# ut-amrl/IV_SLAM

Measured on AMD Instinct MI355X. Metric: stereo pairs/s (extract+match+introspect) @1242×375, 1000 feat; 1/2/4/8 GPU, higher is better.
Workload: dtype u8 (ORB) + f32 via split-f16 MFMA (FCN); 1 GPU; configs[2]: 1242x375 stereo stream with introspection FCN cost-map forward (MFMA convs) gating keypoints, ORB extract + L/R Hamming match; width=1242, height=375, pairs_per_launch_sequence=128, distinct_pairs_per_gpu=512, nfeatures=1000, nlevels=8, parallelism=1 GPU

## Files before the change

### iv_slam_amd/csrc/ivf_fcn.hip

```cpp
#include <hip/hip_runtime.h>
#include <cmath>
#include <cstdarg>
#include <cstdio>
#include <cstdlib>
#include <cstring>
#include <string>
#include <vector>
#include "ivf_device.h"

#define ffail ivf::set_error

#include <type_traits>
namespace ivffcn {

#define FHIP(expr)                                                                                   \
    do { hipError_t e_ = (expr);                                                                      \
         if (e_ != hipSuccess) return ffail(IVF_E_NO_DEVICE, "%s failed: %s", #expr, hipGetErrorString(e_)); } while (0)

typedef float f32x16 __attribute__((ext_vector_type(16)));
typedef float v2f __attribute__((ext_vector_type(2)));
typedef _Float16 f16x8 __attribute__((ext_vector_type(8)));
typedef _Float16 f16x2 __attribute__((ext_vector_type(2)));
union HFrag { f16x8 v; uint4 q; uint32_t u[4]; };
typedef int i32x8 __attribute__((ext_vector_type(8)));
// ... 409 lines not shown
            if (tid + NT * k < NTAB4) ((float4*)sTP)[tid + NT * k] = t4[k];
#pragma unroll
        for (int k = 0; k < IT; k++)
            if (tid + NT * k < N4) *(float4*)&sX[dst[k]] = ok[k] ? v4[k] : make_float4(0.f, 0.f, 0.f, 0.f);
    }
    f32x16 accO;
#pragma unroll
    for (int q = 0; q < 16; q++) accO[q] = 0.f;
    __syncthreads();
    IRB_TIM(0);
    constexpr int TPW = (NTE + 7) / 8;
    HFrag xh[TPW][K16], xl[TPW][K16];
#pragma unroll
    for (int ti = 0; ti < TPW; ti++) {
        const int nc = min(32 * (wv + 8 * ti) + col, NPOS - 1);
        const float* base = sX + (nc / RW) * RP + nc % RW + 3;
#pragma unroll
        for (int st = 0; st < K16; st++)
#pragma unroll
            for (int jj = 0; jj < 4; jj++) {
                const int k0 = 16 * st + 8 * hh + 2 * jj;
                const float x0 = k0 < CIN ? base[k0 * XPL] : 0.f, x1 = k0 + 1 < CIN ? base[(k0 + 1) * XPL] : 0.f;
                split_pair(x0, x1, xh[ti][st].u[jj], xl[ti][st].u[jj]);
            }
    }
    IRB_TIM(1);
#pragma unroll 1
    for (int g = 0; g < NG; g++) {
        HFrag ph[2], pl[2];
        {
            float sc[16], sh[16];
#pragma unroll
            for (int r = 0; r < 16; r++) {
                const float* t = sT + (32 * g + (r & 3) + 8 * (r >> 2) + 4 * hh) * TP;
                sc[r] = t[0]; sh[r] = t[1];
            }
#pragma unroll
            for (int ti = 0; ti < TPW; ti++) {
                const int t = wv + 8 * ti;
                if (t >= NTE) break;
                const int n = 32 * t + col, nc = min(n, NPOS - 1);
                const int r_ = nc / RW, q_ = nc % RW;
                f32x16 acc;
#pragma unroll
                for (int q = 0; q < 16; q++) acc[q] = 0.f;
#pragma unroll
                for (int st = 0; st < K16; st++) {
                    acc = __builtin_amdgcn_mfma_f32_32x32x16_f16(el[st].v, xh[ti][st].v, acc, 0, 0, 0);
                    acc = __builtin_amdgcn_mfma_f32_32x32x16_f16(eh[st].v, xl[ti][st].v, acc, 0, 0, 0);
                    acc = __builtin_amdgcn_mfma_f32_32x32x16_f16(eh[st].v, xh[ti][st].v, acc, 0, 0, 0);
                }
                if (n < NPOS) {
                    const bool edgeWg = ry0 < 0 || rx0 < 0 || ry0 + RH > WI || rx0 + RW > WI;
                    if (!edgeWg) {
#pragma unroll
                        for (int r = 0; r < 16; r++)
                            sH[((r & 3) + 8 * (r >> 2) + 4 * hh) * HPL + n] = __builtin_amdgcn_fmed3f(__builtin_fmaf(acc[r], sc[r], sh[r]), 0.f, 6.f);
                    } else {
                        const bool inside = (unsigned)(ry0 + r_) < (unsigned)WI && (unsigned)(rx0 + q_) < (unsigned)WI;
#pragma unroll
                        for (int r = 0; r < 16; r++) {
                            const float v = __builtin_amdgcn_fmed3f(__builtin_fmaf(acc[r], sc[r], sh[r]), 0.f, 6.f);
                            sH[((r & 3) + 8 * (r >> 2) + 4 * hh) * HPL + n] = inside ? v : 0.f;
                        }
                    }
                }
            }
#ifdef IVF_IRB_ABL_FRAG
            if (g == 0)
#endif
            if (wv < NTP) {
#pragma unroll
                for (int st = 0; st < 2; st++) { ph[st].q = WqP[((2 * g + st) * 2 + 0) * 64 + lane]; pl[st].q = WqP[((2 * g + st) * 2 + 1) * 64 + lane]; }
            }
#ifndef IVF_IRB_ABL_FRAG
            {
                const int gn = g + 1 < NG ? g + 1 : 0;
#pragma unroll
                for (int st = 0; st < K16; st++) { eh[st].q = WqE[((st * NG + gn) * 2 + 0) * 64 + lane]; el[st].q = WqE[((st * NG + gn) * 2 + 1) * 64 + lane]; }
            }
#endif
        }
        IRB_TIM(2);
        __syncthreads();
        IRB_TIM(3);
        {
            const int chl = tid >> 4, sub = tid & 15;
            constexpr int PX = TW * TH / 16;
            const int oy = sub / (TW / PX), x0 = (sub % (TW / PX)) * PX;
            const float* tb = sT + (32 * g + chl) * TP;
            float wk[9];
#pragma unroll
            for (int k = 0; k < 9; k++) wk[k] = tb[2 + k];
            const float dsc = tb[11], dsh = tb[12];
            const float* hp = sH + chl * HPL + (oy * S) * RW + x0 * S;
            float o[PX];
#pragma unroll
            for (int p = 0; p < PX; p++) o[p] = 0.f;
#pragma unroll
            for (int ky = 0; ky < 3; ky++) {
                float row[(PX - 1) * S + 3];
#pragma unroll
                for (int k = 0; k < (PX - 1) * S + 3; k++) row[k] = hp[ky * RW + k];
#pragma unroll
                for (int kx = 0; kx < 3; kx++)
#pragma unroll
                    for (int p = 0; p < PX; p++) o[p] = __builtin_fmaf(wk[ky * 3 + kx], row[p * S + kx], o[p]);
            }
            float* dp = sD + chl * DPL + oy * TW + x0;
#pragma unroll
            for (int p = 0; p < PX; p++) dp[p] = __builtin_amdgcn_fmed3f(__builtin_fmaf(o[p], dsc, dsh), 0.f, 6.f);
        }
        IRB_TIM(4);
        __syncthreads();
        IRB_TIM(5);
        if (wv < NTP) {
            const float* src = sD + 32 * wv + col;
#pragma unroll
            for (int st = 0; st < 2; st++) {
                HFrag bh, bl;
#pragma unroll
                for (int jj = 0; jj < 4; jj++) {
                    const int k0 = 16 * st + 8 * hh + 2 * jj;
                    split_pair(src[k0 * DPL], src[(k0 + 1) * DPL], bh.u[jj], bl.u[jj]);
                }
                accO = __builtin_amdgcn_mfma_f32_32x32x16_f16(pl[st].v, bh.v, accO, 0, 0, 0);
                accO = __builtin_amdgcn_mfma_f32_32x32x16_f16(ph[st].v, bl.v, accO, 0, 0, 0);
                accO = __builtin_amdgcn_mfma_f32_32x32x16_f16(ph[st].v, bh.v, accO, 0, 0, 0);
            }
        }
        IRB_TIM(6);
    }
    if (wv < NTP) {
        const int n = 32 * wv + col, y = oy0 + n / TW, x = ox0 + n % TW;
        float amax = 0.f;
#pragma unroll
        for (int r = 0; r < 16; r++) {
            const int ch = (r & 3) + 8 * (r >> 2) + 4 * hh;
            if (ch >= COUT) continue;
            float v = __builtin_fmaf(accO[r], sPB[ch], sPB[32 + ch]);
            if (RES) v += sX[ch * XPL + (n / TW + 1) * RP + (n % TW + 1) + 3];
            range_note(amax, v);
            Y[(size_t)b * COUT * WO * WO + (ilOut ? ((size_t)y * COUT + ch) * WO : ((size_t)ch * WO + y) * WO) + x] = v;
        }
        range_flag(amax);
    }
#ifdef IVF_IRB_TIMING
    if (WI == IVF_IRB_TIMING && S == IVF_IRB_TIMING_S) {
        asm volatile("s_waitcnt vmcnt(0)" ::: "memory");
        IRB_TIM(7);
        if (tid == 0) { for (int i = 0; i < 8; i++) atomicAdd(&g_irbTim[i], tacc[i]); atomicAdd(&g_irbTim[8], 1ull); }
    }
#endif
}

template <int DIL, int CIN, int HID, int COUT, bool RES>
__global__ __launch_bounds__(512, 4) void k_fcn_irb64(const float* __restrict__ X, const uint4* __restrict__ WqE,
                                                  const float* __restrict__ se, const float* __restrict__ be,
                                                  const float* __restrict__ Wd, const float* __restrict__ sd,
                                                  const float* __restrict__ bd, const uint4* __restrict__ WqP,
                                                  const float* __restrict__ sp, const float* __restrict__ bp, float* __restrict__ Y)
{
    constexpr int NT = 512, WI = 64, TW = 32, TH = 2;
    constexpr int RW = TW + 2 * DIL, RH = TH + 2 * DIL, NPOS = RW * RH;
    constexpr int HPL = (NPOS + 3) / 4 * 4 + 4, DPL = TW * TH + 4;
    constexpr int K16 = (CIN + 15) / 16, NG = (HID + 31) / 32, NTE = (NPOS + 31) / 32, MT = (COUT + 31) / 32, TP = 13;
    static_assert(NTE <= 8, "one window tile per wave");
    static_assert(MT <= 4, "one output-channel tile per wave");
    __shared__ __attribute__((aligned(16))) float sH[32 * HPL];
    __shared__ __attribute__((aligned(16))) float sD[32 * DPL];
    __shared__ float sT[2][32 * TP];
    const int tid = threadIdx.x, b = blockIdx.z;
    const int ox0 = blockIdx.x * TW, oy0 = blockIdx.y * TH;
    const int rx0 = ox0 - DIL, ry0 = oy0 - DIL;
    const float* Xb = X + (size_t)b * CIN * WI * WI;
    const int wv = __builtin_amdgcn_readfirstlane(tid >> 6), lane = tid & 63, hh = lane >> 5, col = lane & 31;
    const float* tsrc; int tstride;
    {
        const int f = tid % TP;
        tsrc = f == 0 ? se : f == 1 ? be : f < 11 ? Wd + (f - 2) : f == 11 ? sd : bd;
        tstride = (f >= 2 && f < 11) ? 9 : 1;
    }
    auto fetch_table = [&](int g) {
        const int c = 32 * g + tid / TP;
        return (tid < 32 * TP && c < HID) ? tsrc[(size_t)c * tstride] : 0.f;
    };
    HFrag eh[K16], el[K16];
#pragma unroll
    for (int st = 0; st < K16; st++) { eh[st].q = WqE[((st * NG + 0) * 2 + 0) * 64 + lane]; el[st].q = WqE[((st * NG + 0) * 2 + 1) * 64 + lane]; }
    if (tid < 32 * TP) sT[0][tid] = fetch_table(0);
    const int n = 32 * wv + col, nc = min(n, NPOS - 1);
    const int r_ = nc / RW, q_ = nc % RW;
    const bool inside = (unsigned)(ry0 + r_) < (unsigned)WI && (unsigned)(rx0 + q_) < (unsigned)WI;
    HFrag xh[K16], xl[K16];
    {
        const float* src = Xb + (size_t)(inside ? ry0 + r_ : 0) * WI + (inside ? rx0 + q_ : 0);
        float xv[K16][8];
#pragma unroll
        for (int st = 0; st < K16; st++)
#pragma unroll
            for (int j = 0; j < 8; j++) {
                const int k = 16 * st + 8 * hh + j;
                xv[st][j] = k < CIN ? src[(size_t)k * WI * WI] : 0.f;
            }
#pragma unroll
        for (int st = 0; st < K16; st++)
#pragma unroll
            for (int jj = 0; jj < 4; jj++)
                split_pair(inside ? xv[st][2 * jj] : 0.f, inside ? xv[st][2 * jj + 1] : 0.f, xh[st].u[jj], xl[st].u[jj]);
    }
    f32x16 accO;
#pragma unroll
    for (int q = 0; q < 16; q++) accO[q] = 0.f;
    const int ntP = wv & 1, mtP = wv >> 1;
    __syncthreads();
#pragma unroll 1
    for (int g = 0; g < NG; g++) {
        const float* T = sT[g & 1];
        const float tnext = g + 1 < NG ? fetch_table(g + 1) : 0.f;
        if (wv < NTE) {
            f32x16 acc, acc1;
#pragma unroll
            for (int q = 0; q < 16; q++) { acc[q] = 0.f; acc1[q] = 0.f; }
#pragma unroll
            for (int st = 0; st < K16; st++) {
                acc1 = __builtin_amdgcn_mfma_f32_32x32x16_f16(el[st].v, xh[st].v, acc1, 0, 0, 0);
                acc = __builtin_amdgcn_mfma_f32_32x32x16_f16(eh[st].v, xh[st].v, acc, 0, 0, 0);
                acc1 = __builtin_amdgcn_mfma_f32_32x32x16_f16(eh[st].v, xl[st].v, acc1, 0, 0, 0);
            }
#pragma unroll
            for (int q = 0; q < 16; q++) acc[q] += acc1[q];
            if (n < NPOS) {
#pragma unroll
                for (int r = 0; r < 16; r++) {
                    const int cl = (r & 3) + 8 * (r >> 2) + 4 * hh;
                    const float v = __builtin_amdgcn_fmed3f(__builtin_fmaf(acc[r], T[cl * TP], T[cl * TP + 1]), 0.f, 6.f);
                    sH[cl * HPL + n] = inside ? v : 0.f;
                }
            }
        }
        if (g + 1 < NG) {
#pragma unroll
            for (int st = 0; st < K16; st++) { eh[st].q = WqE[((st * NG + g + 1) * 2 + 0) * 64 + lane]; el[st].q = WqE[((st * NG + g + 1) * 2 + 1) * 64 + lane]; }
        }
        __syncthreads();
        {
            const int chl = tid >> 4, sub = tid & 15;
            const int oy = sub >> 3, x0 = (sub & 7) * 4;
            const float* tb = T + chl * TP;
            float wk[9];
#pragma unroll
            for (int k = 0; k < 9; k++) wk[k] = tb[2 + k];
            const float dsc = tb[11], dsh = tb[12];
            const float* hp = sH + chl * HPL + oy * RW + x0;
            float o[4] = {0.f, 0.f, 0.f, 0.f};
#pragma unroll
            for (int ky = 0; ky < 3; ky++) {
                float row[4 + 2 * DIL];
#pragma unroll
                for (int k = 0; k < 4 + 2 * DIL; k++) row[k] = hp[ky * DIL * RW + k];
#pragma unroll
                for (int kx = 0; kx < 3; kx++)
#pragma unroll
                    for (int p = 0; p < 4; p++) o[p] = __builtin_fmaf(wk[ky * 3 + kx], row[p + kx * DIL], o[p]);
            }
            float* dp = sD + chl * DPL + oy * TW + x0;
#pragma unroll
            for (int p = 0; p < 4; p++) dp[p] = __builtin_amdgcn_fmed3f(__builtin_fmaf(o[p], dsc, dsh), 0.f, 6.f);
        }
        if (g + 1 < NG && tid < 32 * TP) sT[(g + 1) & 1][tid] = tnext;
        __syncthreads();
        if (mtP < MT) {
            HFrag ph[2], pl[2];
#pragma unroll
            for (int st = 0; st < 2; st++) {
                ph[st].q = WqP[(((2 * g + st) * MT + mtP) * 2 + 0) * 64 + lane];
                pl[st].q = WqP[(((2 * g + st) * MT + mtP) * 2 + 1) * 64 + lane];
            }
            const float* src = sD + 32 * ntP + col;
#pragma unroll
            for (int st = 0; st < 2; st++) {
                HFrag bh, bl;
#pragma unroll
                for (int jj = 0; jj < 4; jj++) {
                    const int k0 = 16 * st + 8 * hh + 2 * jj;
                    split_pair(src[k0 * DPL], src[(k0 + 1) * DPL], bh.u[jj], bl.u[jj]);
                }
                accO = __builtin_amdgcn_mfma_f32_32x32x16_f16(pl[st].v, bh.v, accO, 0, 0, 0);
                accO = __builtin_amdgcn_mfma_f32_32x32x16_f16(ph[st].v, bl.v, accO, 0, 0, 0);
                accO = __builtin_amdgcn_mfma_f32_32x32x16_f16(ph[st].v, bh.v, accO, 0, 0, 0);
            }
        }
    }
    if (mtP < MT) {
        const int m = 32 * ntP + col, y = oy0 + m / TW, x = ox0 + m % TW;
        float amax = 0.f;
#pragma unroll
        for (int r = 0; r < 16; r++) {
            const int ch = 32 * mtP + (r & 3) + 8 * (r >> 2) + 4 * hh;
            if (ch >= COUT) continue;
            float v = __builtin_fmaf(accO[r], sp[ch], bp[ch]);
            if (RES) v += Xb[((size_t)ch * WI + y) * WI + x];
            range_note(amax, v);
            Y[(((size_t)b * COUT + ch) * WI + y) * WI + x] = v;
        }
        range_flag(amax);
// ... 3392 lines not shown
}

int make_fused4(ivf_fcn* f, ivf_fcn::Fused4& F, const float* we, const std::vector<float>& scE, const std::vector<float>& shE, const float* wd,
                const std::vector<float>& scD, const std::vector<float>& shD, const float* wp, int cout, int cin = kF4Cin, int hid = kF4Hid)
{
    const int groups = hid / 16, ksteps = cin / 32;
    auto put = [](uint16_t* q, size_t frag, int lane, int j, float v) {
        const uint16_t hi = f32_to_f16(v), lo = f32_to_f16(v - f16_to_f32(hi));
        q[((frag + 0) * 64 + lane) * 8 + j] = hi; q[((frag + 1) * 64 + lane) * 8 + j] = lo;
    };
    F.cout = cout; F.tilesP = cout / 32;
    std::vector<float> qe((size_t)groups * ksteps * 2 * 64 * 4, 0.f), qp((size_t)groups * F.tilesP * 2 * 64 * 4, 0.f), par((size_t)hid * 12, 0.f);
    uint16_t* e16 = reinterpret_cast<uint16_t*>(qe.data()); uint16_t* p16 = reinterpret_cast<uint16_t*>(qp.data());
    for (int g = 0; g < groups; g++) {
        for (int s5 = 0; s5 < ksteps; s5++)
            for (int lane = 0; lane < 64; lane++)
                for (int j = 0; j < 8; j++)
                    put(e16, ((size_t)g * ksteps + s5) * 2, lane, j, we[(size_t)(16 * g + (lane & 15)) * cin + 32 * s5 + 8 * (lane >> 4) + j]);
        for (int t = 0; t < F.tilesP; t++)
            for (int lane = 0; lane < 64; lane++)
                for (int j = 0; j < 8; j++)
                    put(p16, ((size_t)g * F.tilesP + t) * 2, lane, j, wp[(size_t)(32 * t + (lane & 31)) * hid + 16 * g + 8 * (lane >> 5) + j]);
    }
    for (int c = 0; c < hid; c++) {
        for (int q = 0; q < 9; q++) par[(size_t)c * 12 + q] = wd[(size_t)c * 9 + q] * scD[c];
        par[(size_t)c * 12 + 9] = shD[c]; par[(size_t)c * 12 + 10] = scE[c]; par[(size_t)c * 12 + 11] = shE[c];
    }
    float *de = nullptr, *dp = nullptr;
    int rc;
    if ((rc = upload(f, qe, &de)) || (rc = upload(f, qp, &dp)) || (rc = upload(f, par, &F.dPar))) return rc;
    F.dWE = reinterpret_cast<uint4*>(de); F.dWP = reinterpret_cast<uint4*>(dp);
    if (IVF_F4_FP6_BUILT && cin == kF4Cin && hid == kF4Hid) {
        std::vector<float> q6((size_t)groups * 10 * 64 * 4, 0.f);
        uint32_t* d32 = reinterpret_cast<uint32_t*>(q6.data());
        uint16_t* d16 = reinterpret_cast<uint16_t*>(q6.data());
        for (int g = 0; g < groups; g++) {
            const size_t base = (size_t)g * 10 * 64 * 4;
            for (int s5 = 0; s5 < 5; s5++)
                for (int lane = 0; lane < 64; lane++)
                    for (int j = 0; j < 8; j++)
                        d16[(base + ((size_t)s5 * 64 + lane) * 4) * 2 + j] = f32_to_f16(we[(size_t)(16 * g + (lane & 15)) * cin + 32 * s5 + 8 * (lane >> 4) + j]);
            for (int c = 0; c < 3; c++)
                for (int lane = 0; lane < 64; lane++) {
                    int codes[32];
                    for (int e = 0; e < 32; e++) {
                        const int seg = e >> 3, j = e & 7, s5 = 2 * c + (seg >> 1);
                        float v = 0.f;
                        if (s5 < 5) {
                            const float w = we[(size_t)(16 * g + (lane & 15)) * cin + 32 * s5 + 8 * (lane >> 4) + j];
                            const float hi = f16_to_f32(f32_to_f16(w)), lo = f16_to_f32(f32_to_f16(w - hi));
                            v = (seg & 1) ? std::ldexp(hi, kF6SH) : std::ldexp(lo, kF6SH + 10);
                        }
                        codes[e] = enc6(v, true);
                    }
                    uint32_t six[6]; pack6(six, codes);
                    for (int q = 0; q < 4; q++) d32[base + ((size_t)(5 + c) * 64 + lane) * 4 + q] = six[q];
                    d32[base + (size_t)8 * 64 * 4 + ((size_t)c * 64 + lane) * 2 + 0] = six[4];
                    d32[base + (size_t)8 * 64 * 4 + ((size_t)c * 64 + lane) * 2 + 1] = six[5];
                }
        }
        float* d6 = nullptr;
        if ((rc = upload(f, q6, &d6))) return rc;
        F.dWE6 = reinterpret_cast<uint4*>(d6);
    }
    return IVF_OK;
}

int reserve_lds()
{
    struct { const void* fn; size_t lds; const char* name; } ks[] = {
        {reinterpret_cast<const void*>(&k_fcn_irbd2<32, 32, true, 1>), D2Cfg<32, 32, 1>::LDS, "k_fcn_irbd2<32,32,true,1>"},
        {reinterpret_cast<const void*>(&k_fcn_irbd2<32, 64, false, 1>), D2Cfg<32, 64, 1>::LDS, "k_fcn_irbd2<32,64,false,1>"},
        {reinterpret_cast<const void*>(&k_fcn_irbd2<64, 64, true>), D2Cfg<64, 64>::LDS, "k_fcn_irbd2<64,64,true>"},
        {reinterpret_cast<const void*>(&k_fcn_irbd2<64, 96, false>), D2Cfg<64, 96>::LDS, "k_fcn_irbd2<64,96,false>"},
        {reinterpret_cast<const void*>(&k_fcn_irbd2<96, 96, true>), D2Cfg<96, 96>::LDS, "k_fcn_irbd2<96,96,true>"},
        {reinterpret_cast<const void*>(&k_fcn_irbd2<96, 160, false>), D2Cfg<96, 160>::LDS, "k_fcn_irbd2<96,160,false>"},
        {reinterpret_cast<const void*>(&k_fcn_irbd4<true>), kF4Lds, "k_fcn_irbd4<true>"},
        {reinterpret_cast<const void*>(&k_fcn_irbd4<false>), kF4Lds, "k_fcn_irbd4<false>"},
#if IVF_F4_FP6_BUILT
        {reinterpret_cast<const void*>(&k_fcn_irbd4<true, false, true>), kF4Lds, "k_fcn_irbd4<true,fp6>"},
        {reinterpret_cast<const void*>(&k_fcn_irbd4<false, false, true>), kF4Lds, "k_fcn_irbd4<false,fp6>"},
        {reinterpret_cast<const void*>(&k_fcn_irbd4<false, true, true>), kF4Lds, "k_fcn_irbd4<split,fp6>"},
#endif
        {reinterpret_cast<const void*>(&k_fcn_irbd2<64, 64, true, 2, true>), D2Cfg<64, 64>::LDS, "k_fcn_irbd2<64,64,split>"},
        {reinterpret_cast<const void*>(&k_fcn_irbd2<64, 96, false, 2, true>), D2Cfg<64, 96>::LDS, "k_fcn_irbd2<64,96,split>"},
        {reinterpret_cast<const void*>(&k_fcn_irbd2<96, 96, true, 2, true>), D2Cfg<96, 96>::LDS, "k_fcn_irbd2<96,96,split>"},
        {reinterpret_cast<const void*>(&k_fcn_irbd2<96, 160, false, 2, true>), D2Cfg<96, 160>::LDS, "k_fcn_irbd2<96,160,split>"},
        {reinterpret_cast<const void*>(&k_fcn_irbd4<false, true>), kF4Lds, "k_fcn_irbd4<split>"},
        {reinterpret_cast<const void*>(&k_fcn_irbd4h<false>), kH4Lds, "k_fcn_irbd4h"},
#if IVF_F4_FP6_BUILT
        {reinterpret_cast<const void*>(&k_fcn_irbd4h<true>), kH4Lds, "k_fcn_irbd4h<fp6>"},
#endif
#ifdef IVF_EXPERIMENT
        {reinterpret_cast<const void*>(&k_fcn_irbd4w<true>), kF4Lds, "k_fcn_irbd4w<true>"},
        {reinterpret_cast<const void*>(&k_fcn_irbd4w<false>), kF4Lds, "k_fcn_irbd4w<false>"},
        {reinterpret_cast<const void*>(&k_fcn_irbd4w<false, true>), kF4Lds, "k_fcn_irbd4w<split>"},
#endif
    };
    for (auto& k : ks)
        if (hipFuncSetAttribute(k.fn, hipFuncAttributeMaxDynamicSharedMemorySize, (int)k.lds) != hipSuccess)
            return ffail(IVF_E_NO_DEVICE, "cannot reserve %zu bytes of LDS for %s", k.lds, k.name);
#ifdef IVF_EXPERIMENT
    if (const char* e = IVF_EXP_ENV("IVF_FCN_WABL")) { const int v = atoi(e); FHIP(hipMemcpyToSymbol(HIP_SYMBOL(g_wAbl), &v, sizeof v)); }
#endif
    return IVF_OK;
}

constexpr size_t kPartFloats = (size_t)16 * 320 * 4096;
int split_ways(int n, int groups, int cout)
{
    static const int mode = IVF_EXP_ENV("IVF_FCN_SPLIT") ? atoi(IVF_EXP_ENV("IVF_FCN_SPLIT")) : 1;
    if (!mode || n >= 16) return 1;
    int ns = std::min(16 / n, groups / 4);
    while (ns > 1 && (size_t)ns * n * cout * 4096 > kPartFloats) ns--;
    return std::max(ns, 1);
}
#ifndef IVF_PERSIST
#define IVF_PERSIST 1
#endif
int persistent_grid(const ivf_fcn* f, int tiles)
{
    static const int mode = IVF_EXP_ENV("IVF_FCN_PERSIST") ? atoi(IVF_EXP_ENV("IVF_FCN_PERSIST")) : IVF_PERSIST;
    const int g = f->numCU & ~7;
    return (mode && g >= 8 && tiles >= 2 * g && tiles % 8 == 0) ? g : tiles;
}
void launch_split_reduce(ivf_fcn* f, int ns, int n, int cout, const Gemm& pj, const float* res, float* y, int layIn, int layOut, hipStream_t s)
{
    const size_t total4 = (size_t)n * cout * 1024;
    hipLaunchKernelGGL(k_fcn_split_reduce, dim3((unsigned)((total4 + 255) / 256)), dim3(256), 0, s, (const float*)f->bufPart, ns, (size_t)n * cout * 4096, cout,
                       (const float*)pj.dScale, (const float*)pj.dShift, res, y, total4, layIn, layOut);
}

#define STAGE(name)                                                                                          \
    do { if (dbg) { hipError_t e_ = hipStreamSynchronize(s); if (e_ == hipSuccess) e_ = hipGetLastError();   \
                    fprintf(stderr, "[ivf_fcn] %s: %s\n", name, hipGetErrorString(e_));                      \
                    if (e_ != hipSuccess) return ffail(IVF_E_NO_DEVICE, "stage %s: %s", name, hipGetErrorString(e_)); } } while (0)

int forward_device(ivf_fcn* f, const uint8_t* dBgr, size_t imageStride, int rowStride, int n, uint8_t* dU8, float* dF,
                   hipStream_t s, size_t uImageStride = 0, int uRowStride = 0)
{
    if (!uRowStride) { uRowStride = f->outW; uImageStride = (size_t)f->outW * f->outH; }
    static const bool dbg = getenv("IVF_FCN_DEBUG") != nullptr;
    char nm[64];
    static const int headChunkEnv = IVF_EXP_ENV("IVF_FCN_HEADCHUNK") ? atoi(IVF_EXP_ENV("IVF_FCN_HEADCHUNK")) : IVF_FCN_HEADCHUNK_DEFAULT;
    int headChunk = headChunkEnv;
    if (headChunk <= 0 || headChunk >= n) headChunk = 0;
    if (!headChunk) {
        hipLaunchKernelGGL(k_fcn_prep, dim3(kEnc / 256, kEnc / kPrepRows, n), dim3(256), 0, s, dBgr, imageStride, rowStride, f->inW, f->inH, f->bufIn);
        STAGE("prep");
    }
    static const unsigned irbMask = (IVF_EXP_ENV("IVF_FCN_NOFUSE") || IVF_EXP_ENV("IVF_FCN_NOSTRIDE2")) ? 0u
                                    : IVF_EXP_ENV("IVF_FCN_IRBMASK") ? (unsigned)strtoul(IVF_EXP_ENV("IVF_FCN_IRBMASK"), nullptr, 0) : 7u;
    static const bool stem = IVF_EXP_ENV("IVF_FCN_NOSTEM") == nullptr && IVF_EXP_ENV("IVF_FCN_WIDE256") == nullptr && IVF_EXP_ENV("IVF_FCN_NOFUSE") == nullptr;
    static const int headIlEnv = IVF_EXP_ENV("IVF_FCN_HEAD_IL") ? atoi(IVF_EXP_ENV("IVF_FCN_HEAD_IL")) : IVF_FCN_HEAD_IL_DEFAULT;
    const int headIl = (headIlEnv && stem && (irbMask & 7u) == 7u) ? 1 : 0;
    const bool chunkedHead = headChunk > 0 && stem && (irbMask & 7u) == 7u;
    if (headChunk > 0 && !chunkedHead) {
        hipLaunchKernelGGL(k_fcn_prep, dim3(kEnc / 256, kEnc / kPrepRows, n), dim3(256), 0, s, dBgr, imageStride, rowStride, f->inW, f->inH, f->bufIn);
        STAGE("prep");
    }
    if (chunkedHead) {
        const Dw& d0 = f->dw[0];
        for (int c0 = 0; c0 < n; c0 += headChunk) {
            const int nb = std::min(headChunk, n - c0);
            float* in = f->bufIn + (size_t)c0 * 3 * kEnc * kEnc;
            float* o1 = f->bufB + (size_t)c0 * 16 * 256 * 256;
            float* o2 = f->bufA + (size_t)c0 * 24 * 128 * 128;
            float* o3 = f->bufB + (size_t)c0 * 24 * 128 * 128;
            float* o4 = f->bufA + (size_t)c0 * 32 * 64 * 64;
            hipLaunchKernelGGL(k_fcn_prep, dim3(kEnc / 256, kEnc / kPrepRows, nb), dim3(256), 0, s, dBgr + (size_t)c0 * imageStride, imageStride, rowStride, f->inW, f->inH, in);
            hipLaunchKernelGGL(k_fcn_stem, dim3(kEnc / 2 / kStemTW, kEnc / 2 / kStemTH, nb), dim3(512), 0, s, (const float*)in, f->dConv0W, f->dConv0S,
                               f->dConv0B, d0.dW, d0.dScale, d0.dShift, f->dProj0W, f->pw[0].dScale, f->pw[0].dShift, o1, f->dStemFrag, headIl);
#define IRBC(S_, CIN_, HID_, COUT_, RES_, WI_, TH_, IP_, ID_, X_, Y_, T_)                                                                          \
            hipLaunchKernelGGL((k_fcn_irb<S_, CIN_, HID_, COUT_, RES_, WI_, TH_>), dim3(WI_ / S_ / 32, WI_ / S_ / TH_, nb), dim3(512), 0, s, (const float*)(X_), \
                               (const uint4*)f->dIrbWE[T_], f->pw[IP_].dScale, f->pw[IP_].dShift, f->dw[ID_].dW, f->dw[ID_].dScale, f->dw[ID_].dShift, (const uint4*)f->dIrbWP[T_], \
                               f->pw[IP_ + 1].dScale, f->pw[IP_ + 1].dShift, (Y_), (const float4*)f->dIrbTab[T_], headIl, (T_ < 2 ? headIl : 0))
            IRBC(2, 16, 96, 24, false, 256, IVF_IRB_TH2, 1, 1, o1, o2, 0);
            IRBC(1, 24, 144, 24, true, 128, IVF_IRB_TH3, 3, 2, o2, o3, 1);
            IRBC(2, 24, 144, 32, false, 128, IVF_IRB_TH4, 5, 3, o3, o4, 2);
#undef IRBC
        }
        STAGE("prep + stem + blocks 2-4, chunked");
    } else if (stem) {
        const Dw& d0 = f->dw[0];
        hipLaunchKernelGGL(k_fcn_stem, dim3(kEnc / 2 / kStemTW, kEnc / 2 / kStemTH, n), dim3(512), 0, s, f->bufIn, f->dConv0W, f->dConv0S,
                           f->dConv0B, d0.dW, d0.dScale, d0.dShift, f->dProj0W, f->pw[0].dScale, f->pw[0].dShift, f->bufB, f->dStemFrag, headIl);
        STAGE("stem (conv0 + block 1)");
    } else {
        hipLaunchKernelGGL(k_fcn_conv0, dim3(1, kEnc / 2, n), dim3(256), 0, s, f->bufIn, f->dConv0W, f->dConv0S, f->dConv0B, f->bufA);
        STAGE("conv0");
    }
    static const int fused1 = IVF_EXP_ENV("IVF_FCN_NOFUSE") ? 0 : IVF_EXP_ENV("IVF_FCN_FUSED1") ? atoi(IVF_EXP_ENV("IVF_FCN_FUSED1")) : 1;
    static const int fused2 = IVF_EXP_ENV("IVF_FCN_NOFUSE") ? 0 : IVF_EXP_ENV("IVF_FCN_FUSED2") ? atoi(IVF_EXP_ENV("IVF_FCN_FUSED2")) : 1;
    static const int fused4 = IVF_EXP_ENV("IVF_FCN_NOFUSE") ? 0 : IVF_EXP_ENV("IVF_FCN_FUSED4") ? atoi(IVF_EXP_ENV("IVF_FCN_FUSED4")) : 1;
    static const bool fuseLast = IVF_EXP_ENV("IVF_FCN_NOFUSELAST") == nullptr && IVF_EXP_ENV("IVF_FCN_OLD3X3") == nullptr &&
                                 IVF_EXP_ENV("IVF_FCN_3X3_SPLIT") == nullptr;
    static const int tileMask = IVF_EXP_ENV("IVF_FCN_TILED") ? atoi(IVF_EXP_ENV("IVF_FCN_TILED")) : 6;
    auto whole = [&](int i) {
        if (i >= 4 && i <= 10 && (irbMask >> (i - 1) & 1)) return false;
        if (i >= 4 && i <= 6) return fused1 && f->f1[i - 4].dWE != nullptr;
        if (i >= 7 && i <= 13) return fused2 && f->f2[i - 7].dWE != nullptr;
        if (i >= 14 && i <= 16) return fused4 && f->f4[i - 14].dWE != nullptr;
        return false;
    };
    int lay[18] = {};
    for (int i = 4; i <= 15; i++)
        if (whole(i) && whole(i + 1)) {
            const int want = i + 1 <= 6 ? 1 : i + 1 <= 13 ? 2 : 4;
            if (tileMask & want) lay[i] = want;
        }
    float *x = f->bufA, *y = f->bufB;
    int H = kEnc / 2, W = kEnc / 2;
    size_t ip = 0, id = 0;
    int iFirst = 0;
    if (chunkedHead) { iFirst = 4; ip = 7; id = 4; H = W = 64; }
    for (int i = iFirst; i < 17; i++) {
        const Block& bk = kBlocks[i];
        const int hid = bk.inp * bk.t;
        const float* h = x;
        if (i == 0 && stem) {
            id++; ip++;
            std::swap(x, y);
            continue;
        }
        if (i >= 4 && i <= 10 && (irbMask >> (i - 1) & 1)) {
            const Gemm& ex = f->pw[ip]; const Gemm& pj = f->pw[ip + 1]; const Dw& d = f->dw[id];
#define IRB64(DIL_, CIN_, HID_, COUT_, RES_)                                                                                \
            hipLaunchKernelGGL((k_fcn_irb64<DIL_, CIN_, HID_, COUT_, RES_>), dim3(2, 32, n), dim3(512), 0, s, x, ex.dWq, ex.dScale,      \
                               ex.dShift, d.dW, d.dScale, d.dShift, pj.dWq, pj.dScale, pj.dShift, y)
            if (i == 4 || i == 5) IRB64(1, 32, 192, 32, true);
            else if (i == 6) IRB64(1, 32, 192, 64, false);
            else if (i <= 9) IRB64(2, 64, 384, 64, true);
            else IRB64(2, 64, 384, 96, false);
#undef IRB64
            ip += 2; id++;
            snprintf(nm, sizeof nm, "block %d whole", i + 1); STAGE(nm);
            std::swap(x, y);
            continue;
        }
        if (i >= 1 && i <= 3 && (irbMask >> (i - 1) & 1)) {
            const Gemm& ex = f->pw[ip]; const Gemm& pj = f->pw[ip + 1]; const Dw& d = f->dw[id];
#define IRB(S_, CIN_, HID_, COUT_, RES_, WI_, TH_)                                                                          \
            hipLaunchKernelGGL((k_fcn_irb<S_, CIN_, HID_, COUT_, RES_, WI_, TH_>), dim3(WI_ / S_ / 32, WI_ / S_ / TH_, n), dim3(512), 0, s, x, \
                               (const uint4*)f->dIrbWE[i - 1], ex.dScale, ex.dShift, d.dW, d.dScale, d.dShift, (const uint4*)f->dIrbWP[i - 1], pj.dScale, pj.dShift, y, \
                               (const float4*)f->dIrbTab[i - 1], headIl, (i < 3 ? headIl : 0))
            if (i == 1) IRB(2, 16, 96, 24, false, 256, IVF_IRB_TH2);
            else if (i == 2) IRB(1, 24, 144, 24, true, 128, IVF_IRB_TH3);
            else IRB(2, 24, 144, 32, false, 128, IVF_IRB_TH4);
#undef IRB
            ip += 2; id++;
            H = (H - 1) / d.stride + 1; W = (W - 1) / d.stride + 1;
            snprintf(nm, sizeof nm, "block %d whole", i + 1); STAGE(nm);
            std::swap(x, y);
            continue;
        }
        const int layIn = i >= 1 ? lay[i - 1] : 0, layOut = lay[i];
        if (fused1 && i >= 4 && i <= 6 && f->f1[i - 4].dWE && H == 64 && W == 64) {
            const ivf_fcn::Fused4& F = f->f1[i - 4];
            const Gemm& pj = f->pw[ip + 1];
            bool ok = true;
            auto go = [&](auto kern, size_t lds) {
                hipLaunchKernelGGL(kern, dim3(persistent_grid(f, 16 * n)), dim3(512), lds, s, x, F.dWE, F.dPar, F.dWP, pj.dScale, pj.dShift, bk.res ? x : (const float*)nullptr, y,
                                   (float*)nullptr, layIn, layOut, 16 * n);
            };
            if (bk.oup == 32 && bk.res) go(&k_fcn_irbd2<32, 32, true, 1>, D2Cfg<32, 32, 1>::LDS);
            else if (bk.oup == 64 && !bk.res) go(&k_fcn_irbd2<32, 64, false, 1>, D2Cfg<32, 64, 1>::LDS);
            else ok = false;
            if (!ok) return ffail(IVF_E_NO_DEVICE, "block %d: no k_fcn_irbd2<DIL 1> instance / LDS reservation failed", i + 1);
            ip += 2; id++;
            snprintf(nm, sizeof nm, "block %d whole (4-row strips)", i + 1); STAGE(nm);
            std::swap(x, y);
            continue;
        }
        if (fused2 && i >= 7 && i <= 13 && f->f2[i - 7].dWE && H == 64 && W == 64) {
            const ivf_fcn::Fused4& F = f->f2[i - 7];
            const Gemm& pj = f->pw[ip + 1];
            bool ok = true;
            const int ns = split_ways(n, hid / 16, bk.oup);
            auto go = [&](auto kern, auto kernSplit, size_t lds, bool walk = true) {
                if (ns > 1) {
                    hipLaunchKernelGGL(kernSplit, dim3(16 * n, 1, ns), dim3(512), lds, s, x, F.dWE, F.dPar, F.dWP, pj.dScale, pj.dShift, (const float*)nullptr, y,
                                       f->bufPart, layIn, layOut, 16 * n);
                    launch_split_reduce(f, ns, n, bk.oup, pj, bk.res ? x : nullptr, y, layIn, layOut, s);
                } else
                    hipLaunchKernelGGL(kern, dim3(walk ? persistent_grid(f, 16 * n) : 16 * n), dim3(512), lds, s, x, F.dWE, F.dPar, F.dWP, pj.dScale, pj.dShift,
                                       bk.res ? x : (const float*)nullptr, y, (float*)nullptr, layIn, layOut, 16 * n);
            };
            if (bk.inp == 64 && bk.oup == 64 && bk.res) go(&k_fcn_irbd2<64, 64, true>, &k_fcn_irbd2<64, 64, true, 2, true>, D2Cfg<64, 64>::LDS);
            else if (bk.inp == 64 && bk.oup == 96 && !bk.res) go(&k_fcn_irbd2<64, 96, false>, &k_fcn_irbd2<64, 96, false, 2, true>, D2Cfg<64, 96>::LDS);
            else if (bk.inp == 96 && bk.oup == 96 && bk.res) go(&k_fcn_irbd2<96, 96, true>, &k_fcn_irbd2<96, 96, true, 2, true>, D2Cfg<96, 96>::LDS);
            else if (bk.inp == 96 && bk.oup == 160 && !bk.res) go(&k_fcn_irbd2<96, 160, false>, &k_fcn_irbd2<96, 160, false, 2, true>, D2Cfg<96, 160>::LDS, D2Cfg<96, 160>::WALK);
            else ok = false;
            if (!ok) return ffail(IVF_E_NO_DEVICE, "block %d: no k_fcn_irbd2 instance / LDS reservation failed", i + 1);
            ip += 2; id++;
            snprintf(nm, sizeof nm, "block %d whole (dilation-2 strips)", i + 1); STAGE(nm);
            std::swap(x, y);
            continue;
        }
        if (fused4 && i >= 14 && f->f4[i - 14].dWE && H == 64 && W == 64) {
            const ivf_fcn::Fused4& F = f->f4[i - 14];
            const Gemm& pj = f->pw[ip + 1];
            const bool probe4 = i == 14 && f->probe0[0];
            const int slot4 = (int)(f->probeCount % ivf_fcn::kProbe);
            if (probe4) FHIP(hipEventRecord(f->probe0[slot4], s));
            const bool probeB = i == 16 && f->probeB0[0];
            const int slotB = (int)(f->probeBCount % ivf_fcn::kProbe);
            if (probeB) FHIP(hipEventRecord(f->probeB0[slotB], s));
            const char* kname = "k_fcn_irbd4";
            const int ns = split_ways(n, kF4Groups, F.cout);
            const dim3 grid(16 * n, F.cout / 160, ns);
            static const int fp6 = IVF_EXP_ENV("IVF_FCN_FP6") ? atoi(IVF_EXP_ENV("IVF_FCN_FP6")) : IVF_F4_FP6;
            static const int half4 = IVF_EXP_ENV("IVF_FCN_HALF4") ? atoi(IVF_EXP_ENV("IVF_FCN_HALF4")) : 1;
#ifdef IVF_EXPERIMENT
            static const int roles = IVF_EXP_ENV("IVF_FCN_ROLES") ? atoi(IVF_EXP_ENV("IVF_FCN_ROLES")) : 0;
            if (roles) {
                if (ns > 1) {
                    hipLaunchKernelGGL((k_fcn_irbd4w<false, true>), grid, dim3(1024), kF4Lds, s, x, F.dWE, F.dPar, F.dWP, pj.dScale, pj.dShift, (const float*)nullptr, y,
                                       F.cout, F.tilesP, f->bufPart, layIn, layOut);
                    launch_split_reduce(f, ns, n, F.cout, pj, bk.res ? x : nullptr, y, layIn, layOut, s);
                } else if (bk.res)
                    hipLaunchKernelGGL((k_fcn_irbd4w<true>), grid, dim3(1024), kF4Lds, s, x, F.dWE, F.dPar, F.dWP, pj.dScale, pj.dShift, x, y, F.cout, F.tilesP, (float*)nullptr,
                                       layIn, layOut);
                else
                    hipLaunchKernelGGL((k_fcn_irbd4w<false>), grid, dim3(1024), kF4Lds, s, x, F.dWE, F.dPar, F.dWP, pj.dScale, pj.dShift, (const float*)nullptr, y, F.cout, F.tilesP,
                                       (float*)nullptr, layIn, layOut);
            } else
#endif
            if (ns > 1) {
#if IVF_F4_FP6_BUILT
                if (fp6 && F.dWE6)
                    hipLaunchKernelGGL((k_fcn_irbd4<false, true, true>), grid, dim3(512), kF4Lds, s, x, F.dWE6, F.dPar, F.dWP, pj.dScale, pj.dShift, (const float*)nullptr, y,
                                       F.cout, F.tilesP, f->bufPart, layIn, layOut, 16 * n);
                else
#endif
                hipLaunchKernelGGL((k_fcn_irbd4<false, true>), grid, dim3(512), kF4Lds, s, x, F.dWE, F.dPar, F.dWP, pj.dScale, pj.dShift, (const float*)nullptr, y,
                                   F.cout, F.tilesP, f->bufPart, layIn, layOut, 16 * n);
                launch_split_reduce(f, ns, n, F.cout, pj, bk.res ? x : nullptr, y, layIn, layOut, s);
            } else if (half4 && !bk.res && F.cout == kH4Cout && F.tilesP == kH4TilesP)
            {
#if IVF_F4_FP6_BUILT
                if (fp6 && F.dWE6)
                    hipLaunchKernelGGL(k_fcn_irbd4h<true>, dim3(32 * n), dim3(512), kH4Lds, s, x, F.dWE6, F.dPar, F.dWP, pj.dScale, pj.dShift, y, layIn, layOut, 32 * n);
                else
#endif
                hipLaunchKernelGGL(k_fcn_irbd4h<false>, dim3(IVF_H4_WALK ? persistent_grid(f, 32 * n) : 32 * n), dim3(512), kH4Lds, s, x, F.dWE, F.dPar, F.dWP, pj.dScale, pj.dShift, y,
                                   layIn, layOut, 32 * n);
                kname = "k_fcn_irbd4h";
            }
#if IVF_F4_FP6_BUILT
            else if (fp6 && F.dWE6 && bk.res)
                hipLaunchKernelGGL((k_fcn_irbd4<true, false, true>), dim3(16 * n, grid.y, 1), dim3(512), kF4Lds, s, x, F.dWE6, F.dPar, F.dWP, pj.dScale,
                                   pj.dShift, x, y, F.cout, F.tilesP, (float*)nullptr, layIn, layOut, 16 * n);
            else if (fp6 && F.dWE6)
                hipLaunchKernelGGL((k_fcn_irbd4<false, false, true>), grid, dim3(512), kF4Lds, s, x, F.dWE6, F.dPar, F.dWP, pj.dScale, pj.dShift, (const float*)nullptr, y, F.cout, F.tilesP,
                                   (float*)nullptr, layIn, layOut, 16 * n);
#endif
            else if (bk.res)
                hipLaunchKernelGGL((k_fcn_irbd4<true>), dim3(IVF_F4_WALK && grid.y == 1 ? persistent_grid(f, 16 * n) : 16 * n, grid.y, 1), dim3(512), kF4Lds, s, x, F.dWE, F.dPar, F.dWP, pj.dScale,
                                   pj.dShift, x, y, F.cout, F.tilesP, (float*)nullptr, layIn, layOut, 16 * n);
            else
                hipLaunchKernelGGL((k_fcn_irbd4<false>), grid, dim3(512), kF4Lds, s, x, F.dWE, F.dPar, F.dWP, pj.dScale, pj.dShift, (const float*)nullptr, y, F.cout, F.tilesP,
                                   (float*)nullptr, layIn, layOut, 16 * n);
            if (probe4) {
                FHIP(hipEventRecord(f->probe1[slot4], s)); f->probeBatch[slot4] = n; f->probeCount++;
                snprintf(f->probeName, sizeof f->probeName, "ivffcn::k_fcn_irbd4<%s> %d->%d->%d", bk.res ? "true" : "false", bk.inp, hid, bk.oup);
                f->probeAlgoBytes = (double)(bk.inp + bk.oup) * H * W * sizeof(float);
            }
            if (probeB) {
                FHIP(hipEventRecord(f->probeB1[slotB], s)); f->probeBCount++;
                if (strcmp(kname, "k_fcn_irbd4h") == 0) snprintf(f->probeBName, sizeof f->probeBName, "ivffcn::k_fcn_irbd4h %d->%d->%d", bk.inp, hid, bk.oup);
                else snprintf(f->probeBName, sizeof f->probeBName, "ivffcn::k_fcn_irbd4<%s> %d->%d->%d", bk.res ? "true" : "false", bk.inp, hid, bk.oup);
                f->probeBAlgoBytes = (double)(bk.inp + bk.oup) * H * W * sizeof(float);
            }
            ip += 2; id++;
            snprintf(nm, sizeof nm, "block %d whole (dilation-4 phases)", i + 1); STAGE(nm);
            std::swap(x, y);
            continue;
        }
        static const int chunkEnv = IVF_EXP_ENV("IVF_FCN_CHUNK") ? atoi(IVF_EXP_ENV("IVF_FCN_CHUNK")) : 0;
        if (chunkEnv > 0 && bk.t != 1 && H == 64 && W == 64 && n > chunkEnv && bk.stride == 1) {
            const Dw& d = f->dw[id];
            bool ok = true;
            for (int c0 = 0; c0 < n && ok; c0 += chunkEnv) {
                const int nb = std::min(chunkEnv, n - c0);
                const float* xo = x + (size_t)c0 * bk.inp * H * W;
                float* yo = y + (size_t)c0 * bk.oup * H * W;
                if (!launch_expand(f->pw[ip], xo, f->bufH1, H, W, nb, s)) launch_gemm(f->pw[ip], xo, nullptr, f->bufH1, H, W, nb, s);
                ok = launch_dwpw(d, f->pw[ip + 1], f->bufH1, bk.res ? xo : nullptr, yo, H, W, nb, s);
            }
            if (!ok) return ffail(IVF_E_STATE, "chunked schedule: block %d has no fused depthwise + projection kernel", i + 1);
            ip += 2; id++;
            snprintf(nm, sizeof nm, "block %d chunked", i + 1); STAGE(nm);
            std::swap(x, y);
            continue;
        }
        if (bk.t != 1) {
            if (!launch_expand(f->pw[ip], x, f->bufH1, H, W, n, s)) launch_gemm(f->pw[ip], x, nullptr, f->bufH1, H, W, n, s);
            ip++; h = f->bufH1; snprintf(nm, sizeof nm, "block %d expand", i + 1); STAGE(nm); }
        const Dw& d = f->dw[id++];
        const bool probe = i == 14 && f->probe0[0];
        const int slot = (int)(f->probeCount % ivf_fcn::kProbe);
// ... 439 lines not shown
```

Before: 11990 pairs/s.

## Add software-pipelined IRB kernel interleaving expand, depthwise and projection by half-groups

Adds a new fused inverted-residual kernel for the three stride/early blocks. It processes the hidden channels in 16-channel halves, so the expand MFMA, depthwise 3x3 and projection MFMA of successive halves overlap across loop iterations. sH and sD are double-buffered and weights are prefetched one step ahead. Folded per-channel parameters come from a single table copied to LDS, and launch bounds are derived from the LDS footprint. The new kernel is the default, with an env flag to fall back to the old one; the cost is more barriers per block and extra register pressure from held accumulators.

```diff
diff --git a/iv_slam_amd/csrc/ivf_fcn.hip b/iv_slam_amd/csrc/ivf_fcn.hip
--- a/iv_slam_amd/csrc/ivf_fcn.hip
+++ b/iv_slam_amd/csrc/ivf_fcn.hip
@@ -585,6 +585,245 @@
         if (tid == 0) { for (int i = 0; i < 8; i++) atomicAdd(&g_irbTim[i], tacc[i]); atomicAdd(&g_irbTim[8], 1ull); }
     }
 #endif
+}
+
+#ifndef IVF_IRBI_TH2
+#define IVF_IRBI_TH2 2
+#endif
+#ifndef IVF_IRBI_TH3
+#define IVF_IRBI_TH3 4
+#endif
+#ifndef IVF_IRBI_TH4
+#define IVF_IRBI_TH4 4
+#endif
+constexpr int irbi_waves(int S, int CIN, int TH)
+{
+    const int RW = 31 * S + 3, RH = (TH - 1) * S + 3, NPOS = RW * RH, XPL = RH * 4 * ((RW + 6) / 4) + 4;
+    const int HPL = S == 1 ? (NPOS + 15) / 32 * 32 + 16 : (NPOS | 1), DPL = 32 * TH + 16;
+    const int bytes = 4 * (CIN * XPL + 32 * HPL + 32 * DPL + (CIN == 16 ? 3 : 5) * 32 * 13 + 64);
+    return bytes <= 80 * 1024 ? 4 : 2;
+}
+template <int S, int CIN, int HID, int COUT, bool RES, int WI, int TH>
+__global__ __launch_bounds__(512, irbi_waves(S, CIN, TH)) void k_fcn_irbi(const float* __restrict__ X, const uint4* __restrict__ WqE_, const uint4* __restrict__ WqP_,
+                                                 float* __restrict__ Y, const float4* __restrict__ tab4, int ilIn, int ilOut)
+{
+    constexpr int NT = 512, WO = WI / S, TW = 32;
+    constexpr int RW = (TW - 1) * S + 3, RH = (TH - 1) * S + 3, NPOS = RW * RH;
+    constexpr int Q4 = (RW + 3 + 3) / 4, RP = 4 * Q4, XPL = RH * RP + 4;
+    constexpr int HPL = S == 1 ? (NPOS + 15) / 32 * 32 + 16 : (NPOS | 1), DPL = TW * TH + 16;
+    static_assert(TW * TH % 32 == 0 && DPL % 32 == 16, "sD planes: 16 banks apart");
+    constexpr int K16 = (CIN + 15) / 16, NG = (HID + 31) / 32, NH = HID / 16, NTE = (NPOS + 31) / 32, NTP = TW * TH / 32;
+    static_assert(HID % 16 == 0 && NTP <= 8, "16-channel halves, at most one projection tile per wave");
+    constexpr int TP = 13, NI = NH + 2;
+    constexpr int TPW = (NTE + 7) / 8;
+    __shared__ __attribute__((aligned(16))) float sX[CIN * XPL];
+    __shared__ __attribute__((aligned(16))) float sH[2 * 16 * HPL];
+    __shared__ __attribute__((aligned(16))) float sD[2 * 16 * DPL];
+    constexpr int NTAB = NG * 32 * TP + 64, NTAB4 = NTAB / 4, ITT = (NTAB4 + NT - 1) / NT;
+    static_assert(NTAB % 4 == 0, "table is copied in 16-byte pieces");
+    __shared__ __attribute__((aligned(16))) float sTP[NTAB];
+    float* const sT = sTP;
+    float* const sPB = sTP + NG * 32 * TP;
+    const int tid = threadIdx.x, b = blockIdx.z;
+    const int ox0 = blockIdx.x * TW, oy0 = blockIdx.y * TH;
+    const int rx0 = ox0 * S - 1, ry0 = oy0 * S - 1;
+    const float* Xb = X + (size_t)b * CIN * WI * WI;
+    const int wv = __builtin_amdgcn_readfirstlane(tid >> 6), lane = tid & 63, hh = lane >> 5, col = lane & 31;
+    const int pt = 7 - wv;
+    const uint4* WqE = WqE_; const uint4* WqP = WqP_;
+    {
+        const unsigned lin = blockIdx.x + gridDim.x * (blockIdx.y + gridDim.y * blockIdx.z);
+        const unsigned rep_ = (lin >> 3) % (unsigned)kIrbRep;
+        WqE += (size_t)rep_ * (K16 * NG * 128);
+        WqP += (size_t)rep_ * (2 * NG * 128);
+    }
+    HFrag eh[K16], el[K16];
+#pragma unroll
+    for (int st = 0; st < K16; st++) { eh[st].q = WqE[((st * NG + 0) * 2 + 0) * 64 + lane]; el[st].q = WqE[((st * NG + 0) * 2 + 1) * 64 + lane]; }
+    HFrag ph[2], pl[2];
+    {
+        constexpr int N4 = CIN * RH * Q4, IT = (N4 + NT - 1) / NT;
+        float4 v4[IT]; bool ok[IT]; int dst[IT];
+        constexpr int DC = NT / (RH * Q4), DR = (NT % (RH * Q4)) / Q4, DQ = NT % Q4;
+        int c = tid / (RH * Q4), r = (tid / Q4) % RH, q4 = tid % Q4;
+#pragma unroll
+        for (int k = 0; k < IT; k++) {
+            if (k > 0) {
+                q4 += DQ; const int cq = q4 >= Q4 ? 1 : 0; q4 -= cq * Q4;
+                r += DR + cq; const int cr = r >= RH ? 1 : 0; r -= cr * RH;
+                c = min(c + DC + cr, CIN - 1);
+            }
+            const int yy = ry0 + r, xx = ox0 * S - 4 + 4 * q4;
+            ok[k] = yy >= 0 && yy < WI && xx >= 0 && xx < WI;
+            dst[k] = c * XPL + r * RP + 4 * q4;
+            v4[k] = *(const float4*)(Xb + (ilIn ? ((size_t)(ok[k] ? yy : 0) * CIN + c) * WI : ((size_t)c * WI + (ok[k] ? yy : 0)) * WI) + (ok[k] ? xx : 0));
+        }
+        float4 t4[ITT];
+#pragma unroll
+        for (int k = 0; k < ITT; k++) t4[k] = tab4[min(tid + NT * k, NTAB4 - 1)];
+#pragma unroll
+        for (int k = 0; k < ITT; k++) asm volatile("" : "+v"(t4[k].x), "+v"(t4[k].y), "+v"(t4[k].z), "+v"(t4[k].w));
+#pragma unroll
+        for (int k = 0; k < IT; k++) asm volatile("" : "+v"(v4[k].x), "+v"(v4[k].y), "+v"(v4[k].z), "+v"(v4[k].w));
+        __builtin_amdgcn_sched_barrier(0);
+#pragma unroll
+        for (int k = 0; k < ITT; k++)
+            if (tid + NT * k < NTAB4) ((float4*)sTP)[tid + NT * k] = t4[k];
+#pragma unroll
+        for (int k = 0; k < IT; k++)
+            if (tid + NT * k < N4) *(float4*)&sX[dst[k]] = ok[k] ? v4[k] : make_float4(0.f, 0.f, 0.f, 0.f);
+    }
+    f32x16 accO;
+#pragma unroll
+    for (int q = 0; q < 16; q++) accO[q] = 0.f;
+    __syncthreads();
+    HFrag xh[TPW][K16], xl[TPW][K16];
+#pragma unroll
+    for (int ti = 0; ti < TPW; ti++) {
+        const int nc = min(32 * (wv + 8 * ti) + col, NPOS - 1);
+        const float* base = sX + (nc / RW) * RP + nc % RW + 3;
+#pragma unroll
+        for (int st = 0; st < K16; st++)
+#pragma unroll
+            for (int jj = 0; jj < 4; jj++) {
+                const int k0 = 16 * st + 8 * hh + 2 * jj;
+                const float x0 = k0 < CIN ? base[k0 * XPL] : 0.f, x1 = k0 + 1 < CIN ? base[(k0 + 1) * XPL] : 0.f;
+                split_pair(x0, x1, xh[ti][st].u[jj], xl[ti][st].u[jj]);
+            }
+    }
+    const bool edgeWg = ry0 < 0 || rx0 < 0 || ry0 + RH > WI || rx0 + RW > WI;
+    const int sc_ = 4 * (wv >> 1) + (lane >> 4), sx_ = 16 * (wv & 1) + (lane & 15);
+    float hold[TPW][8];
+#pragma unroll
+    for (int i = 0; i < NI; i++) {
+        if (i >= 2) {
+            HFrag& a = ph[i & 1]; HFrag& c = pl[i & 1];
+            asm volatile("" :: "v"(a.q.x), "v"(a.q.y), "v"(a.q.z), "v"(a.q.w), "v"(c.q.x), "v"(c.q.y), "v"(c.q.z), "v"(c.q.w));
+        }
+        if (i % 2 == 0 && i < NH && i > 0)
+#pragma unroll
+            for (int st = 0; st < K16; st++) asm volatile("" :: "v"(eh[st].q.x), "v"(eh[st].q.y), "v"(eh[st].q.z), "v"(eh[st].q.w),
+                                                                "v"(el[st].q.x), "v"(el[st].q.y), "v"(el[st].q.z), "v"(el[st].q.w));
+        if (i >= 1 && i - 1 < NH) { const int hn = i - 1; ph[hn & 1].q = WqP[(hn * 2 + 0) * 64 + lane]; pl[hn & 1].q = WqP[(hn * 2 + 1) * 64 + lane]; }
+        if (i % 2 == 1 && i + 1 < NH) {
+            const int gn = (i + 1) / 2;
+#pragma unroll
+            for (int st = 0; st < K16; st++) { eh[st].q = WqE[((st * NG + gn) * 2 + 0) * 64 + lane]; el[st].q = WqE[((st * NG + gn) * 2 + 1) * 64 + lane]; }
+        }
+        if (i < NH) {
+            float* const hb = sH + (i & 1) * 16 * HPL;
+            if (i % 2 == 0) {
+                const int g = i / 2;
+                float sc[8], sh[8];
+#pragma unroll
+                for (int r = 0; r < 8; r++) {
+                    const float* t = sT + (32 * g + (r & 3) + 8 * (r >> 2) + 4 * hh) * TP;
+                    sc[r] = t[0]; sh[r] = t[1];
+                }
+#pragma unroll
+                for (int ti = 0; ti < TPW; ti++) {
+                    const int t = wv + 8 * ti;
+                    if (t >= NTE) break;
+                    const int n = 32 * t + col, nc = min(n, NPOS - 1);
+                    const int r_ = nc / RW, q_ = nc % RW;
+                    f32x16 acc;
+#pragma unroll
+                    for (int q = 0; q < 16; q++) acc[q] = 0.f;
+#pragma unroll
+                    for (int st = 0; st < K16; st++) {
+                        acc = __builtin_amdgcn_mfma_f32_32x32x16_f16(el[st].v, xh[ti][st].v, acc, 0, 0, 0);
+                        acc = __builtin_amdgcn_mfma_f32_32x32x16_f16(eh[st].v, xl[ti][st].v, acc, 0, 0, 0);
+                        acc = __builtin_amdgcn_mfma_f32_32x32x16_f16(eh[st].v, xh[ti][st].v, acc, 0, 0, 0);
+                    }
+                    const bool inside = !edgeWg || ((unsigned)(ry0 + r_) < (unsigned)WI && (unsigned)(rx0 + q_) < (unsigned)WI);
+                    if (n < NPOS)
+#pragma unroll
+                        for (int r = 0; r < 8; r++) {
+                            const float v = __builtin_amdgcn_fmed3f(__builtin_fmaf(acc[r], sc[r], sh[r]), 0.f, 6.f);
+                            hb[((r & 3) + 8 * (r >> 2) + 4 * hh) * HPL + n] = inside ? v : 0.f;
+                        }
+#pragma unroll
+                    for (int r = 0; r < 8; r++) hold[ti][r] = acc[8 + r];
+                }
+            } else {
+                const int g = i / 2;
+                float sc[8], sh[8];
+#pragma unroll
+                for (int r = 0; r < 8; r++) {
+                    const float* t = sT + (32 * g + 16 + (r & 3) + 8 * (r >> 2) + 4 * hh) * TP;
+                    sc[r] = t[0]; sh[r] = t[1];
+                }
+#pragma unroll
+                for (int ti = 0; ti < TPW; ti++) {
+                    const int t = wv + 8 * ti;
+                    if (t >= NTE) break;
+                    const int n = 32 * t + col, nc = min(n, NPOS - 1);
+                    const bool inside = !edgeWg || ((unsigned)(ry0 + nc / RW) < (unsigned)WI && (unsigned)(rx0 + nc % RW) < (unsigned)WI);
+                    if (n < NPOS)
+#pragma unroll
+                        for (int r = 0; r < 8; r++) {
+                            const float v = __builtin_amdgcn_fmed3f(__builtin_fmaf(hold[ti][r], sc[r], sh[r]), 0.f, 6.f);
+                            hb[((r & 3) + 8 * (r >> 2) + 4 * hh) * HPL + n] = inside ? v : 0.f;
+                        }
+                }
+            }
+        }
+        if (i >= 1 && i <= NH) {
+            const int h = i - 1;
+            const float* tb = sT + (16 * h + sc_) * TP;
+            float wk[9];
+#pragma unroll
+            for (int k = 0; k < 9; k++) wk[k] = tb[2 + k];
+            const float dsc = tb[11], dsh = tb[12];
+            const float* hp = sH + (h & 1) * 16 * HPL + sc_ * HPL + sx_ * S;
+            float o[TH];
+#pragma unroll
+            for (int p = 0; p < TH; p++) o[p] = 0.f;
+#pragma unroll
+            for (int R = 0; R < RH; R++) {
+                const float h0 = hp[R * RW], h1 = hp[R * RW + 1], h2 = hp[R * RW + 2];
+#pragma unroll
+                for (int p = 0; p < TH; p++) {
+                    const int ky = R - S * p;
+                    if (ky < 0 || ky > 2) continue;
+                    o[p] = __builtin_fmaf(wk[ky * 3 + 0], h0, o[p]);
+                    o[p] = __builtin_fmaf(wk[ky * 3 + 1], h1, o[p]);
+                    o[p] = __builtin_fmaf(wk[ky * 3 + 2], h2, o[p]);
+                }
+            }
+            float* dp = sD + (h & 1) * 16 * DPL + sc_ * DPL + sx_;
+#pragma unroll
+            for (int p = 0; p < TH; p++) dp[p * TW] = __builtin_amdgcn_fmed3f(__builtin_fmaf(o[p], dsc, dsh), 0.f, 6.f);
+        }
+        if (i >= 2 && pt < NTP) {
+            const int h = i - 2;
+            const float* src = sD + (h & 1) * 16 * DPL + 32 * pt + col;
+            HFrag bh, bl;
+#pragma unroll
+            for (int jj = 0; jj < 4; jj++) {
+                const int k0 = 8 * hh + 2 * jj;
+                split_pair(src[k0 * DPL], src[(k0 + 1) * DPL], bh.u[jj], bl.u[jj]);
+            }
+            accO = __builtin_amdgcn_mfma_f32_32x32x16_f16(pl[h & 1].v, bh.v, accO, 0, 0, 0);
+            accO = __builtin_amdgcn_mfma_f32_32x32x16_f16(ph[h & 1].v, bl.v, accO, 0, 0, 0);
+            accO = __builtin_amdgcn_mfma_f32_32x32x16_f16(ph[h & 1].v, bh.v, accO, 0, 0, 0);
+        }
+        if (i + 1 < NI) __syncthreads();
+    }
+    if (pt < NTP) {
+        const int n = 32 * pt + col, y = oy0 + n / TW, x = ox0 + n % TW;
+        float amax = 0.f;
+#pragma unroll
+        for (int r = 0; r < 16; r++) {
+            const int ch = (r & 3) + 8 * (r >> 2) + 4 * hh;
+            if (ch >= COUT) continue;
+            float v = __builtin_fmaf(accO[r], sPB[ch], sPB[32 + ch]);
+            if (RES) v += sX[ch * XPL + (n / TW + 1) * RP + (n % TW + 1) + 3];
+            range_note(amax, v);
+            Y[(size_t)b * COUT * WO * WO + (ilOut ? ((size_t)y * COUT + ch) * WO : ((size_t)ch * WO + y) * WO) + x] = v;
+        }
+        range_flag(amax);
+    }
 }
 
 template <int DIL, int CIN, int HID, int COUT, bool RES>
@@ -4283,6 +4522,7 @@
     static const unsigned irbMask = (IVF_EXP_ENV("IVF_FCN_NOFUSE") || IVF_EXP_ENV("IVF_FCN_NOSTRIDE2")) ? 0u
                                     : IVF_EXP_ENV("IVF_FCN_IRBMASK") ? (unsigned)strtoul(IVF_EXP_ENV("IVF_FCN_IRBMASK"), nullptr, 0) : 7u;
     static const bool stem = IVF_EXP_ENV("IVF_FCN_NOSTEM") == nullptr && IVF_EXP_ENV("IVF_FCN_WIDE256") == nullptr && IVF_EXP_ENV("IVF_FCN_NOFUSE") == nullptr;
+    static const bool irbOld = IVF_EXP_ENV("IVF_FCN_IRB_OLD") != nullptr;
     static const int headIlEnv = IVF_EXP_ENV("IVF_FCN_HEAD_IL") ? atoi(IVF_EXP_ENV("IVF_FCN_HEAD_IL")) : IVF_FCN_HEAD_IL_DEFAULT;
     const int headIl = (headIlEnv && stem && (irbMask & 7u) == 7u) ? 1 : 0;
     const bool chunkedHead = headChunk > 0 && stem && (irbMask & 7u) == 7u;
@@ -4306,9 +4546,19 @@
             hipLaunchKernelGGL((k_fcn_irb<S_, CIN_, HID_, COUT_, RES_, WI_, TH_>), dim3(WI_ / S_ / 32, WI_ / S_ / TH_, nb), dim3(512), 0, s, (const float*)(X_), \
                                (const uint4*)f->dIrbWE[T_], f->pw[IP_].dScale, f->pw[IP_].dShift, f->dw[ID_].dW, f->dw[ID_].dScale, f->dw[ID_].dShift, (const uint4*)f->dIrbWP[T_], \
                                f->pw[IP_ + 1].dScale, f->pw[IP_ + 1].dShift, (Y_), (const float4*)f->dIrbTab[T_], headIl, (T_ < 2 ? headIl : 0))
-            IRBC(2, 16, 96, 24, false, 256, IVF_IRB_TH2, 1, 1, o1, o2, 0);
-            IRBC(1, 24, 144, 24, true, 128, IVF_IRB_TH3, 3, 2, o2, o3, 1);
-            IRBC(2, 24, 144, 32, false, 128, IVF_IRB_TH4, 5, 3, o3, o4, 2);
+#define IRBIC(S_, CIN_, HID_, COUT_, RES_, WI_, TH_, X_, Y_, T_)                                                                              \
+            hipLaunchKernelGGL((k_fcn_irbi<S_, CIN_, HID_, COUT_, RES_, WI_, TH_>), dim3(WI_ / S_ / 32, WI_ / S_ / TH_, nb), dim3(512), 0, s, (const float*)(X_), \
+                               (const uint4*)f->dIrbWE[T_], (const uint4*)f->dIrbWP[T_], (Y_), (const float4*)f->dIrbTab[T_], headIl, (T_ < 2 ? headIl : 0))
+            if (irbOld) {
+                IRBC(2, 16, 96, 24, false, 256, IVF_IRB_TH2, 1, 1, o1, o2, 0);
+                IRBC(1, 24, 144, 24, true, 128, IVF_IRB_TH3, 3, 2, o2, o3, 1);
+                IRBC(2, 24, 144, 32, false, 128, IVF_IRB_TH4, 5, 3, o3, o4, 2);
+            } else {
+                IRBIC(2, 16, 96, 24, false, 256, IVF_IRBI_TH2, o1, o2, 0);
+                IRBIC(1, 24, 144, 24, true, 128, IVF_IRBI_TH3, o2, o3, 1);
+                IRBIC(2, 24, 144, 32, false, 128, IVF_IRBI_TH4, o3, o4, 2);
+            }
+#undef IRBIC
 #undef IRBC
         }
         STAGE("prep + stem + blocks 2-4, chunked");
@@ -4375,9 +4625,19 @@
             hipLaunchKernelGGL((k_fcn_irb<S_, CIN_, HID_, COUT_, RES_, WI_, TH_>), dim3(WI_ / S_ / 32, WI_ / S_ / TH_, n), dim3(512), 0, s, x, \
                                (const uint4*)f->dIrbWE[i - 1], ex.dScale, ex.dShift, d.dW, d.dScale, d.dShift, (const uint4*)f->dIrbWP[i - 1], pj.dScale, pj.dShift, y, \
                                (const float4*)f->dIrbTab[i - 1], headIl, (i < 3 ? headIl : 0))
-            if (i == 1) IRB(2, 16, 96, 24, false, 256, IVF_IRB_TH2);
-            else if (i == 2) IRB(1, 24, 144, 24, true, 128, IVF_IRB_TH3);
-            else IRB(2, 24, 144, 32, false, 128, IVF_IRB_TH4);
+#define IRBI(S_, CIN_, HID_, COUT_, RES_, WI_, TH_)                                                                         \
+            hipLaunchKernelGGL((k_fcn_irbi<S_, CIN_, HID_, COUT_, RES_, WI_, TH_>), dim3(WI_ / S_ / 32, WI_ / S_ / TH_, n), dim3(512), 0, s, x, \
+                               (const uint4*)f->dIrbWE[i - 1], (const uint4*)f->dIrbWP[i - 1], y, (const float4*)f->dIrbTab[i - 1], headIl, (i < 3 ? headIl : 0))
+            if (irbOld) {
+                if (i == 1) IRB(2, 16, 96, 24, false, 256, IVF_IRB_TH2);
+                else if (i == 2) IRB(1, 24, 144, 24, true, 128, IVF_IRB_TH3);
+                else IRB(2, 24, 144, 32, false, 128, IVF_IRB_TH4);
+            } else {
+                if (i == 1) IRBI(2, 16, 96, 24, false, 256, IVF_IRBI_TH2);
+                else if (i == 2) IRBI(1, 24, 144, 24, true, 128, IVF_IRBI_TH3);
+                else IRBI(2, 24, 144, 32, false, 128, IVF_IRBI_TH4);
+            }
+#undef IRBI
 #undef IRB
             ip += 2; id++;
             H = (H - 1) / d.stride + 1; W = (W - 1) / d.stride + 1;
```

Result: no change. 12060 pairs/s, median of 6 (+0.6%).
